# mjsargent/gym-miniworld

Measured on AMD Instinct MI355X. Metric: env-steps/s (80x60 RGB obs), higher is better.
Workload: dtype f64 sim / f32 render / u8 obs; 1 GPU; maze8192; env_id=MiniWorld-Maze-v0, envs_per_gpu=8192, global_envs=8192, obs=80x60 RGB, domain_rand=False, actions=uniform random over {turn_left, turn_right, move_forward}, counter-based, auto_reset=True, parallelism=env-sharded x1

## Files before the change

### gym_miniworld_amd/build.py

```python
import os
import subprocess
import sys

HERE = os.path.dirname(os.path.abspath(__file__))
CSRC = os.path.join(HERE, "csrc")
SOURCES = ["mwb_api.hip", "mwb_kernels.hip"]
HEADERS = ["mwb_internal.h", "mwb_glibc_trig.h", "mwb_sincos_table.inc", os.path.join("..", "..", "include", "miniworld_batch.h")]
OUT = os.path.join(HERE, "libmwbatch.so")
REMARKS = os.path.join(HERE, "libmwbatch.resources.txt")
FLAGS = ["--offload-arch=gfx950", "-O3", "-std=c++17", "-fPIC", "-shared", "-ffp-contract=off", "-Wall",
         "-Wno-unused-value"]


def needs_build():
    if not os.path.exists(OUT):
        return True
    t = os.path.getmtime(OUT)
    return any(os.path.getmtime(os.path.join(CSRC, f)) > t for f in SOURCES + HEADERS)


def source_digest():
    import hashlib
    h = hashlib.sha1()
    for f in SOURCES + HEADERS:
        with open(os.path.join(CSRC, f), "rb") as fh:
            h.update(fh.read())
    h.update(" ".join(FLAGS).encode())
    return h.hexdigest()


def build(force=False, verbose=False):
    if not force and not needs_build():
        return OUT
    hipcc = os.environ.get("HIPCC", "/opt/rocm/bin/hipcc")
    if not os.path.exists(hipcc):
        hipcc = "hipcc"
    cmd = [hipcc] + FLAGS + ["-Rpass-analysis=kernel-resource-usage", "-o", OUT] + [os.path.join(CSRC, f) for f in SOURCES]
    if verbose:
        print(" ".join(cmd))
    digest = source_digest()
    r = subprocess.run(cmd, stderr=subprocess.PIPE, text=True)
    remarks = [ln for ln in r.stderr.split("\n") if "-Rpass-analysis" in ln]
    rest = [ln for ln in r.stderr.split("\n") if "-Rpass-analysis" not in ln and ln.strip()]
    if rest:
        sys.stderr.write("\n".join(rest) + "\n")
    if r.returncode != 0:
        raise subprocess.CalledProcessError(r.returncode, cmd)
    with open(REMARKS, "w") as fh:
        fh.write("digest %s\n" % digest)
        fh.write("\n".join(remarks) + "\n")
    return OUT


if __name__ == "__main__":
    build(force="--force" in sys.argv, verbose=True)
    print("built", OUT)
```

### gym_miniworld_amd/csrc/mwb_api.hip

```cpp
#include <math.h>
#include <stdio.h>
#include <stdlib.h>
#include <string.h>

#include <string>
#include <vector>

#include "mwb_internal.h"

static thread_local std::string g_err;
static int set_err(int code, const std::string &msg) { g_err = msg; return code; }
#define HIP_TRY(expr)                                                                       \
    do {                                                                                    \
        hipError_t _e = (expr);                                                             \
        if (_e != hipSuccess)                                                               \
            return set_err(MWB_EHIP, std::string(#expr) + ": " + hipGetErrorString(_e));    \
    } while (0)

struct DevGuard {
    int prev = -1;
    hipError_t err;
    explicit DevGuard(int dev) {
        err = hipGetDevice(&prev);
        if (err == hipSuccess && prev != dev) err = hipSetDevice(dev); else if (err == hipSuccess) prev = -1;
    }
    ~DevGuard() { if (prev >= 0) (void)hipSetDevice(prev); }
};
#define USE_DEVICE(dev)                                                                             \
    DevGuard _dev_guard(dev);                                                                        \
    if (_dev_guard.err != hipSuccess)                                                                \
        return set_err(MWB_EHIP, std::string("hipSetDevice: ") + hipGetErrorString(_dev_guard.err))

struct mwb_handle {
    mwb_config cfg;
    MwbDev dev;
    std::vector<void *> allocs;
    std::vector<std::vector<uint32_t>> tex_levels[MWB_MAX_TEX];
    int tex_w[MWB_MAX_TEX], tex_h[MWB_MAX_TEX];
    uint32_t *texels_dev;
    MwbTexDesc *tex_desc_dev;
    bool seeded, textures_dirty, have_textures;
    bool have_obs;
    int *scratch_int_dev;
    bool timing, timing_now;
    int timing_period, timing_tick;
    std::vector<hipEvent_t> ev_pool;
    size_t ev_used;
    hipEvent_t *ev;
    bool overlap_reset;
    void *pack;
    size_t pack_bytes;
    void *stack;
    int stack_n, stack_dtype;
    int stack_fused;
    int stack_planes, stack_pos;
    size_t stack_bytes;
    hipStream_t side;
    hipEvent_t ev_fork, ev_join;
    struct HostMesh { bool set = false; int n_tris = 0, n_nodes = 0, n_orders = 1, tex_id = -1; float min_c[3], max_c[3]; std::vector<float> nodes, tris, tris2, shade; };
    HostMesh meshes[MWB_NUM_MESHES];
    bool meshes_dirty;
    float4 *mesh_data_dev;
    MwbMeshDesc *mesh_desc_dev;
    float *view_frame;
    bool frame_reuse;
};

extern "C" const char *mwb_last_error(void) { return g_err.c_str(); }
extern "C" int mwb_abi_version(void) { return MWB_ABI_VERSION; }

static const uint64_t K512[80] = {
    0x428a2f98d728ae22ULL, 0x7137449123ef65cdULL, 0xb5c0fbcfec4d3b2fULL, 0xe9b5dba58189dbbcULL, 0x3956c25bf348b538ULL,
    0x59f111f1b605d019ULL, 0x923f82a4af194f9bULL, 0xab1c5ed5da6d8118ULL, 0xd807aa98a3030242ULL, 0x12835b0145706fbeULL,
    0x243185be4ee4b28cULL, 0x550c7dc3d5ffb4e2ULL, 0x72be5d74f27b896fULL, 0x80deb1fe3b1696b1ULL, 0x9bdc06a725c71235ULL,
    0xc19bf174cf692694ULL, 0xe49b69c19ef14ad2ULL, 0xefbe4786384f25e3ULL, 0x0fc19dc68b8cd5b5ULL, 0x240ca1cc77ac9c65ULL,
    0x2de92c6f592b0275ULL, 0x4a7484aa6ea6e483ULL, 0x5cb0a9dcbd41fbd4ULL, 0x76f988da831153b5ULL, 0x983e5152ee66dfabULL,
    0xa831c66d2db43210ULL, 0xb00327c898fb213fULL, 0xbf597fc7beef0ee4ULL, 0xc6e00bf33da88fc2ULL, 0xd5a79147930aa725ULL,
    0x06ca6351e003826fULL, 0x142929670a0e6e70ULL, 0x27b70a8546d22ffcULL, 0x2e1b21385c26c926ULL, 0x4d2c6dfc5ac42aedULL,
    0x53380d139d95b3dfULL, 0x650a73548baf63deULL, 0x766a0abb3c77b2a8ULL, 0x81c2c92e47edaee6ULL, 0x92722c851482353bULL,
    0xa2bfe8a14cf10364ULL, 0xa81a664bbc423001ULL, 0xc24b8b70d0f89791ULL, 0xc76c51a30654be30ULL, 0xd192e819d6ef5218ULL,
    0xd69906245565a910ULL, 0xf40e35855771202aULL, 0x106aa07032bbd1b8ULL, 0x19a4c116b8d2d0c8ULL, 0x1e376c085141ab53ULL,
    0x2748774cdf8eeb99ULL, 0x34b0bcb5e19b48a8ULL, 0x391c0cb3c5c95a63ULL, 0x4ed8aa4ae3418acbULL, 0x5b9cca4f7763e373ULL,
    0x682e6ff3d6b2b8a3ULL, 0x748f82ee5defb2fcULL, 0x78a5636f43172f60ULL, 0x84c87814a1f0ab72ULL, 0x8cc702081a6439ecULL,
    0x90befffa23631e28ULL, 0xa4506cebde82bde9ULL, 0xbef9a3f7b2c67915ULL, 0xc67178f2e372532bULL, 0xca273eceea26619cULL,
    0xd186b8c721c0c207ULL, 0xeada7dd6cde0eb1eULL, 0xf57d4f7fee6ed178ULL, 0x06f067aa72176fbaULL, 0x0a637dc5a2c898a6ULL,
    0x113f9804bef90daeULL, 0x1b710b35131c471bULL, 0x28db77f523047d84ULL, 0x32caab7b40c72493ULL, 0x3c9ebe0a15c9bebcULL,
    0x431d67c49c100d4cULL, 0x4cc5d4becb3e42b6ULL, 0x597f299cfc657e2aULL, 0x5fcb6fab3ad6faecULL, 0x6c44198c4a475817ULL};

static inline uint64_t rotr64(uint64_t x, int n) { return (x >> n) | (x << (64 - n)); }

static void sha512_short(const uint8_t *msg, size_t len, uint8_t out[64]) {
// ... 229 lines not shown
    if (rc == MWB_OK && (d.exp_flags & 4)) rc = dev_alloc(h, &d.dbg_counters, (size_t)8);
    if (rc == MWB_OK) rc = dev_alloc(h, &d.cost, 2 * N);
    if (rc == MWB_OK) rc = dev_alloc(h, &d.bucket, N);
    if (rc == MWB_OK) rc = dev_alloc(h, &d.order_bufs[0], N);
    if (rc == MWB_OK) rc = dev_alloc(h, &d.order_bufs[1], N);
    if (rc == MWB_OK) rc = dev_alloc(h, &d.order_state, (size_t)2);
    if (rc == MWB_OK) {
        std::vector<int32_t> ident(N);
        for (size_t i = 0; i < N; i++) ident[i] = (int32_t)i;
        for (int k = 0; k < 2 && rc == MWB_OK; k++)
            if (hipMemcpy(d.order_bufs[k], ident.data(), N * sizeof(int32_t), hipMemcpyHostToDevice) != hipSuccess) rc = set_err(MWB_EHIP, "mwb_create: hipMemcpy failed");
    }
    if (rc != MWB_OK) { mwb_destroy(h); return rc; }
    if ((d.task == MWB_TASK_TMAZE && d.task_args[3] > 0) || (d.task == MWB_TASK_TMAZE_TWOBOX && d.task_args[0] == 0)) {
        std::vector<int64_t> ones(N, 1);
        if (hipMemcpy(d.episode_count, ones.data(), N * sizeof(int64_t), hipMemcpyHostToDevice) != hipSuccess) {
            mwb_destroy(h);
            return set_err(MWB_EHIP, "mwb_create: hipMemcpy failed");
        }
    }
    if (hipMemset(d.carrying, 0xFF, N * sizeof(int32_t)) != hipSuccess) { mwb_destroy(h); return set_err(MWB_EHIP, "mwb_create: hipMemset failed"); }
    d.tex_desc = h->tex_desc_dev;
    h->texels_dev = nullptr; d.texels = nullptr;
    h->seeded = false; h->textures_dirty = false; h->have_textures = false; h->have_obs = false;
    h->timing = false; h->timing_now = false; h->timing_period = 1; h->timing_tick = 0; h->ev_used = 0; h->ev = nullptr;
    { const char *no = getenv("MWB_NO_OVERLAP"); h->overlap_reset = !(no && atoi(no)); }
    h->side = nullptr; h->ev_fork = nullptr; h->ev_join = nullptr;
    h->view_frame = nullptr;
    h->meshes_dirty = false; h->mesh_data_dev = nullptr; d.mesh_desc = h->mesh_desc_dev; d.mesh_data = nullptr;
    h->stack = nullptr; h->stack_n = 0; h->stack_dtype = 0; h->stack_bytes = 0; h->stack_planes = 0; h->stack_pos = 0; h->stack_fused = 0;
    int prio_lo = 0, prio_hi = 0;
    hipDeviceGetStreamPriorityRange(&prio_lo, &prio_hi);
    if (hipStreamCreateWithPriority(&h->side, hipStreamNonBlocking, prio_hi) != hipSuccess ||
        hipEventCreateWithFlags(&h->ev_fork, hipEventDisableTiming) != hipSuccess ||
        hipEventCreateWithFlags(&h->ev_join, hipEventDisableTiming) != hipSuccess) {
        mwb_destroy(h);
        return set_err(MWB_EHIP, "mwb_create: could not create the side stream / events");
    }
    for (int i = 0; i < MWB_MAX_TEX; i++) { h->tex_w[i] = 0; h->tex_h[i] = 0; }
    if (d.tile_w == 0) {
        int wshift = 0;
        while ((1 << wshift) < d.W) wshift++;
        if (mwb_render_lds_bytes(d) > 160 * 1024 || ((size_t)d.H << wshift) > 65536) {
            int tw = 0, th = 0;
            mwb_view_tile(&tw, &th);
            d.tile_w = tw < d.W ? tw : d.W; d.tile_h = th < d.H ? th : d.H;
        }
    }
    { const char *no = getenv("MWB_NO_FRAME_REUSE"); h->frame_reuse = !(no && atoi(no)) && d.tile_w == 0; }
    rc = dev_alloc(h, &d.reuse_stats, (size_t)2);
    if (rc == MWB_OK && h->frame_reuse) {
        rc = dev_alloc(h, &d.frame_cache, N * d.W * d.H * 3);
        if (rc == MWB_OK && d.want_depth) rc = dev_alloc(h, &d.depth_cache, N * d.W * d.H);
        if (rc == MWB_OK) rc = dev_alloc(h, &d.frame_cached, N);
        if (rc == MWB_OK) rc = dev_alloc(h, &d.frame_same, N);
    }
    if (rc != MWB_OK) { mwb_destroy(h); return rc; }
    if (int prc = mwb_prepare_kernels(d)) {
        mwb_destroy(h);
        return set_err(prc == -2 ? MWB_EHIP : MWB_EINVAL,
                       prc == -1 ? "mwb_create: world + observation too large for the 160 KB LDS staging buffers (room table + W*H*3 frame)"
                       : prc == -3 ? "mwb_create: observation too large for the 16-bit pixel queue (H << ceil(log2 W) must not exceed 65536)"
                                   : "mwb_create: hipFuncSetAttribute(MaxDynamicSharedMemorySize) failed");
    }
    *out = h;
    return MWB_OK;
}

extern "C" int mwb_destroy(mwb_handle *h) {
    if (!h) return MWB_OK;
    DevGuard _dev_guard(h->cfg.device);
    hipDeviceSynchronize();
    for (void *p : h->allocs) hipFree(p);
    if (h->texels_dev) hipFree(h->texels_dev);
    if (h->mesh_data_dev) hipFree(h->mesh_data_dev);
    for (hipEvent_t e : h->ev_pool) hipEventDestroy(e);
    if (h->ev_fork) hipEventDestroy(h->ev_fork);
    if (h->ev_join) hipEventDestroy(h->ev_join);
    if (h->side) hipStreamDestroy(h->side);
    delete h;
    return MWB_OK;
}

static void build_mips(const uint8_t *rgb, int w, int h, std::vector<std::vector<uint32_t>> &levels) {
    levels.clear();
    std::vector<uint32_t> cur((size_t)w * h);
    for (int y = 0; y < h; y++)
        for (int x = 0; x < w; x++) {
            const uint8_t *p = rgb + ((size_t)(h - 1 - y) * w + x) * 3;
            cur[(size_t)y * w + x] = p[0] | (p[1] << 8) | (p[2] << 16) | 0xFF000000u;
        }
    levels.push_back(cur);
    int sw = w, sh = h;
    while (sw > 1 || sh > 1) {
        int dw = sw > 1 ? sw / 2 : 1, dh = sh > 1 ? sh / 2 : 1;
        std::vector<uint32_t> nxt((size_t)dw * dh);
        const std::vector<uint32_t> &src = levels.back();
        for (int j = 0; j < dh; j++) {
            int j0 = (int)(((long long)j * sh) / dh), j1 = (int)((((long long)(j + 1) * sh) + dh - 1) / dh);
            for (int i = 0; i < dw; i++) {
                int i0 = (int)(((long long)i * sw) / dw), i1 = (int)((((long long)(i + 1) * sw) + dw - 1) / dw);
                uint32_t sum[4] = {0, 0, 0, 0};
                for (int y = j0; y < j1; y++)
                    for (int x = i0; x < i1; x++) {
                        uint32_t t = src[(size_t)y * sw + x];
                        sum[0] += t & 255u; sum[1] += (t >> 8) & 255u; sum[2] += (t >> 16) & 255u; sum[3] += t >> 24;
                    }
                uint32_t cnt = (uint32_t)((j1 - j0) * (i1 - i0));
                uint32_t o = 0;
                for (int c = 0; c < 4; c++) o |= ((sum[c] + cnt / 2) / cnt) << (8 * c);
                nxt[(size_t)j * dw + i] = o;
            }
        }
        levels.push_back(nxt);
        sw = dw; sh = dh;
    }
}

extern "C" int mwb_set_texture(mwb_handle *h, int tex_id, int width, int height, const uint8_t *rgb) {
    if (!h || !rgb) return set_err(MWB_EINVAL, "mwb_set_texture: null argument");
    if (tex_id < 0 || tex_id >= MWB_MAX_TEX || width <= 0 || height <= 0 || width > 4096 || height > 4096)
        return set_err(MWB_EINVAL, "mwb_set_texture: bad texture id or size");
    build_mips(rgb, width, height, h->tex_levels[tex_id]);
    if ((int)h->tex_levels[tex_id].size() > MWB_MAX_LEVELS) return set_err(MWB_EINVAL, "mwb_set_texture: too many mip levels");
    h->tex_w[tex_id] = width; h->tex_h[tex_id] = height;
    h->textures_dirty = true;
    return MWB_OK;
}

static int upload_textures(mwb_handle *h) {
    USE_DEVICE(h->cfg.device);
    const int n_tex = h->dev.n_tex;
    for (int i = 0; i < n_tex; i++)
        if (h->tex_w[i] == 0)
            return set_err(MWB_ESTATE, "render requested before the task's " + std::to_string(n_tex) + " textures were set (mwb_set_texture)");
    std::vector<uint32_t> all;
    MwbTexDesc desc[MWB_MAX_TEX];
    memset(desc, 0, sizeof(desc));
    for (int i = 0; i < n_tex; i++) {
        desc[i].w = h->tex_w[i]; desc[i].h = h->tex_h[i]; desc[i].n_levels = (int)h->tex_levels[i].size();
        desc[i].sc_s = (float)(512.0 / h->tex_w[i]); desc[i].sc_t = (float)(512.0 / h->tex_h[i]);
        for (size_t l = 0; l < h->tex_levels[i].size(); l++) {
            desc[i].level_off[l] = (uint32_t)all.size();
            all.insert(all.end(), h->tex_levels[i][l].begin(), h->tex_levels[i][l].end());
        }
    }
    HIP_TRY(hipDeviceSynchronize());
    if (h->texels_dev) { hipFree(h->texels_dev); h->texels_dev = nullptr; }
    HIP_TRY(hipMalloc((void **)&h->texels_dev, all.size() * 4));
    HIP_TRY(hipMemcpy(h->texels_dev, all.data(), all.size() * 4, hipMemcpyHostToDevice));
    HIP_TRY(hipMemcpy(h->tex_desc_dev, desc, sizeof(desc), hipMemcpyHostToDevice));
    h->dev.texels = h->texels_dev;
    h->textures_dirty = false; h->have_textures = true;
    return MWB_OK;
}

extern "C" int mwb_set_mesh(mwb_handle *h, int geom, int n_tris, const float *verts, const float *norms, const float *texcs, int tex_slot,
                            const float *min_coords, const float *max_coords, int n_nodes, int n_orders, const float *nodes, const int32_t *perm) {
    if (!h || !verts || !norms || !texcs || !min_coords || !max_coords || !nodes || !perm) return set_err(MWB_EINVAL, "mwb_set_mesh: null argument");
    if (geom < 0 || geom >= MWB_NUM_MESHES || n_tris <= 0 || n_tris >= (1 << 24) || n_nodes <= 0 || tex_slot >= MWB_MAX_TEX || (n_orders != 1 && n_orders != 8))
        return set_err(MWB_EINVAL, "mwb_set_mesh: bad geometry id / sizes");
    for (int ord = 0; ord < n_orders; ord++) {
        std::vector<char> seen((size_t)n_tris, 0);
        const float *on = nodes + (size_t)ord * n_nodes * 8;
        for (int i = 0; i < n_nodes; i++) {
            int32_t skip, fc;
            memcpy(&skip, on + (size_t)i * 8 + 3, 4); memcpy(&fc, on + (size_t)i * 8 + 7, 4);
            const int cnt = (int)((uint32_t)fc >> 24), first = (int)((uint32_t)fc & 0xFFFFFFu);
            if (skip <= i || skip > n_nodes || first + cnt > n_tris || (cnt == 0 && i + 1 >= n_nodes))
                return set_err(MWB_EINVAL, "mwb_set_mesh: malformed hierarchy");
            for (int k = 0; k < cnt; k++) seen[(size_t)first + k] = 1;
        }
        for (int i = 0; i < n_tris; i++)
            if (!seen[i] || perm[i] < 0 || perm[i] >= n_tris) return set_err(MWB_EINVAL, "mwb_set_mesh: the leaves must cover every triangle once");
    }
    mwb_handle::HostMesh &m = h->meshes[geom];
    m.set = true; m.n_tris = n_tris; m.n_nodes = n_nodes; m.n_orders = n_orders; m.tex_id = tex_slot;
    for (int k = 0; k < 3; k++) { m.min_c[k] = min_coords[k]; m.max_c[k] = max_coords[k]; }
    m.nodes.assign(nodes, nodes + (size_t)n_orders * n_nodes * 8);
    auto rec = [&](int tri, float *o) {
        const float *v = verts + (size_t)tri * 9;
        const float e1[3] = {v[3] - v[0], v[4] - v[1], v[5] - v[2]}, e2[3] = {v[6] - v[0], v[7] - v[1], v[8] - v[2]};
        o[0] = v[0]; o[1] = v[1]; o[2] = v[2]; o[3] = e1[0]; o[4] = e1[1]; o[5] = e1[2]; o[6] = e2[0]; o[7] = e2[1]; o[8] = e2[2];
        int32_t idx = tri; memcpy(o + 9, &idx, 4); o[10] = 0; o[11] = 0;
    };
    m.tris.resize((size_t)n_tris * 12); m.tris2.resize((size_t)n_tris * 12); m.shade.assign((size_t)n_tris * 16, 0.0f);
    for (int i = 0; i < n_tris; i++) {
        rec(perm[i], &m.tris[(size_t)i * 12]);
        rec(i, &m.tris2[(size_t)i * 12]);
        float *o = &m.shade[(size_t)i * 16];
        memcpy(o, norms + (size_t)i * 9, 36);
        memcpy(o + 9, texcs + (size_t)i * 6, 24);
    }
    h->meshes_dirty = true;
    return MWB_OK;
}

extern "C" int mwb_set_mesh_dims(mwb_handle *h, int geom, double height, double scale, double radius, int is_f32) {
    if (!h) return set_err(MWB_EINVAL, "mwb_set_mesh_dims: null handle");
    if (geom < 0 || geom >= MWB_NUM_MESHES || !(height > 0) || !(scale > 0) || !(radius > 0) || !std::isfinite(scale) || !std::isfinite(radius))
        return set_err(MWB_EINVAL, "mwb_set_mesh_dims: bad argument");
    MwbDev &d = h->dev;
    int k = 0;
    while (k < d.n_mesh_dims && !(d.mesh_dims[k].geom == geom && d.mesh_dims[k].height == height)) k++;
    if (k == MWB_MAX_MESH_DIMS) return set_err(MWB_EINVAL, "mwb_set_mesh_dims: table full");
    d.mesh_dims[k].geom = geom; d.mesh_dims[k].height = height; d.mesh_dims[k].scale = scale; d.mesh_dims[k].radius = radius; d.mesh_dims[k].is_f32 = is_f32 ? 1 : 0;
    if (k == d.n_mesh_dims) d.n_mesh_dims++;
    return MWB_OK;
}

static const int *task_meshes(int task, int *n) {
    static const int pick[2] = {MWB_MESH_BALL, MWB_MESH_KEY}, health[1] = {MWB_MESH_MEDKIT}, three[3] = {MWB_MESH_DUCKIE, MWB_MESH_KEY, MWB_MESH_BALL},
                     sign[1] = {MWB_MESH_KEY}, side[2] = {MWB_MESH_BUILDING, MWB_MESH_CONE}, gap[1] = {MWB_MESH_BUILDING};
    switch (task) {
    case MWB_TASK_PICKUPOBJS: case MWB_TASK_ROOMOBJS: *n = 2; return pick;
    case MWB_TASK_COLLECTHEALTH: *n = 1; return health;
    case MWB_TASK_THREEROOMS: *n = 3; return three;
    case MWB_TASK_SIGN: *n = 1; return sign;
    case MWB_TASK_SIDEWALK: *n = 2; return side;
    case MWB_TASK_WALLGAP: *n = 1; return gap;
    }
    *n = 0; return nullptr;
}

static int upload_meshes(mwb_handle *h) {
    int n_need = 0;
    const int *need = task_meshes(h->dev.task, &n_need);
    for (int k = 0; k < n_need; k++) {
// ... 684 lines not shown
```

### gym_miniworld_amd/csrc/mwb_kernels.hip

```cpp
#include "mwb_internal.h"
#include "mwb_glibc_trig.h"

#define WAVE 64

__device__ __forceinline__ double ref_sin(double x) { return mwb_trig::in_range(x) ? mwb_trig::sin_glibc(x) : sin(x); }
__device__ __forceinline__ double ref_cos(double x) { return mwb_trig::in_range(x) ? mwb_trig::cos_glibc(x) : cos(x); }

__device__ __forceinline__ uint32_t mt_temper(uint32_t y) {
    y ^= (y >> 11);
    y ^= (y << 7) & 0x9d2c5680u;
    y ^= (y << 15) & 0xefc60000u;
    y ^= (y >> 18);
    return y;
}

__device__ __forceinline__ uint32_t mt_mix(uint32_t a, uint32_t b, uint32_t c) {
    uint32_t y = (a & 0x80000000u) | (b & 0x7fffffffu);
    return c ^ (y >> 1) ^ ((y & 1u) ? 0x9908b0dfu : 0u);
}

struct MtSerial {
    uint32_t *key;
    int pos;
    __device__ void load(uint32_t *st) { key = st; pos = (int)st[624]; }
// ... 1976 lines not shown
        float tmin = t1 < t2 ? t1 : t2, tmax = t1 < t2 ? t2 : t1;
        if (tmin > tn) { tn = tmin; face = a * 2 + (ld[a] > 0 ? 0 : 1); }
        if (tmax < tf) tf = tmax;
    }
    if (miss || face < 0 || !(tn <= tf) || !(tn > 0)) return -1;
    t_out = tn;
    return face;
}

#ifndef ENT_WGS_PER_CU
#define ENT_WGS_PER_CU 4
#endif
#define KIND_MESH 5u
#define KIND_FRAME 6u
__device__ __forceinline__ float dot3f(const float *a, const float *b) { return fmaf(a[2], b[2], fmaf(a[1], b[1], a[0] * b[0])); }
__device__ __forceinline__ void cross3f(const float *a, const float *b, float *o) {
    o[0] = fmaf(a[1], b[2], -(a[2] * b[1])); o[1] = fmaf(a[2], b[0], -(a[0] * b[2])); o[2] = fmaf(a[0], b[1], -(a[1] * b[0]));
}
__device__ __forceinline__ void mesh_local_dir(const float *blk, const float *dv, float *ld) {
    const float c = blk[FC_BOX_C], s = blk[FC_BOX_S], inv_s = blk[FC_LIT_BOX + FE_MESH_INVS];
    ld[0] = fmaf(dv[0], c, -(dv[2] * s)) * inv_s; ld[1] = dv[1] * inv_s; ld[2] = fmaf(dv[0], s, dv[2] * c) * inv_s;
}
__device__ __forceinline__ bool mesh_tri(const float *lo, const float *ld, const float4 r0, const float4 r1, const float4 r2, bool need_inside,
                                         float &t, float &u, float &v, float &det) {
    const float v0[3] = {r0.x, r0.y, r0.z}, e1[3] = {r0.w, r1.x, r1.y}, e2[3] = {r1.z, r1.w, r2.x};
    float pv[3], qv[3];
    cross3f(ld, e2, pv);
    det = dot3f(e1, pv);
    if (!(det > 0.0f)) return false;
    const float tv[3] = {lo[0] - v0[0], lo[1] - v0[1], lo[2] - v0[2]};
    u = dot3f(tv, pv);
    cross3f(tv, e1, qv);
    v = dot3f(ld, qv);
    if (need_inside && (u < 0.0f || u > det || v < 0.0f || u + v > det)) return false;
    t = dot3f(e2, qv) / det;
    return need_inside ? t > 0.0f : true;
}
#define MQ_CAP 320
#define MB_HALF 4
#define MB_TASKS 320
#define MB_WAVE_BYTES (MB_HALF * 64 * 8 + MB_TASKS * 2 + 64 * 4 + 16)
typedef float f4n __attribute__((ext_vector_type(4)));
__device__ __forceinline__ int trace_frame(const float *blk, const float *dv, float &t_out) {
    const float c = blk[FC_BOX_C], s = blk[FC_BOX_S];
    const float *fe = blk + FC_LIT_BOX;
    const float ld[3] = {fmaf(dv[0], c, -(dv[2] * s)), dv[1], fmaf(dv[0], s, dv[2] * c)};
    const float lo_[3] = {blk[FC_BOX_LO], blk[FC_BOX_LO + 1], blk[FC_BOX_LO + 2]};
    const float lo[3] = {0.0f, -fe[FE_FRAME_HY], -fe[FE_FRAME_HZ]}, hi[3] = {fe[FE_FRAME_SX], fe[FE_FRAME_HY], fe[FE_FRAME_HZ]};
    float tn = -INFINITY, tf = INFINITY;
    int face = -1;
    bool miss = false;
#pragma unroll
    for (int a = 0; a < 3; a++) {
        if (ld[a] == 0) { miss = miss || lo_[a] < lo[a] || lo_[a] > hi[a]; continue; }
        const float inv = 1.0f / ld[a];
        const float t1 = (lo[a] - lo_[a]) * inv, t2 = (hi[a] - lo_[a]) * inv;
        const float tmin = t1 < t2 ? t1 : t2, tmax = t1 < t2 ? t2 : t1;
        if (tmin > tn) { tn = tmin; face = a * 2 + (ld[a] > 0 ? 0 : 1); }
        if (tmax < tf) tf = tmax;
    }
    if (miss || face <= 0 || !(tn <= tf) || !(tn > 0)) return -1;
    t_out = tn;
    if (face != 1) return 100;
    const float z = fmaf(tn, ld[2], lo_[2]);
    const int n_ch = __float_as_int(fe[FE_FRAME_NCH]);
    int i = (int)floorf((fe[FE_FRAME_HZ] - z) / fe[FE_FRAME_CW]);
    return i < 0 ? 0 : (i >= n_ch ? n_ch - 1 : i);
}
__device__ __forceinline__ bool frame_front_tc(const float *blk, int cell, const float *dv, float &s_, float &t_) {
    const float c = blk[FC_BOX_C], s = blk[FC_BOX_S];
    const float *fe = blk + FC_LIT_BOX;
    const float ld[3] = {fmaf(dv[0], c, -(dv[2] * s)), dv[1], fmaf(dv[0], s, dv[2] * c)};
    const float lo_[3] = {blk[FC_BOX_LO], blk[FC_BOX_LO + 1], blk[FC_BOX_LO + 2]};
    const float tt = (fe[FE_FRAME_SX] - lo_[0]) / ld[0];
    const float y = fmaf(tt, ld[1], lo_[1]), z = fmaf(tt, ld[2], lo_[2]);
    const float z1 = fe[FE_FRAME_HZ] - fe[FE_FRAME_CW] * (float)cell;
    s_ = (z1 - z) / fe[FE_FRAME_CW]; t_ = (y + fe[FE_FRAME_HY]) / (2.0f * fe[FE_FRAME_HY]);
    return ld[0] != 0.0f && tt > 0.0f;
}

struct TexLds { int w, h, n_levels; float sc_s, sc_t; int pad[3]; uint32_t off[MWB_MAX_LEVELS]; };
static_assert(sizeof(TexLds) == sizeof(MwbTexDesc), "TexLds mirrors MwbTexDesc");

__device__ __forceinline__ void bilinear(const uint32_t *__restrict__ texels, uint32_t off, int w, int h, float s, float t, float *rgb) {
    float uu = fmaf(s, (float)w, -0.5f), vv = fmaf(t, (float)h, -0.5f);
    float fu = floorf(uu), fv = floorf(vv);
    float a = uu - fu, b = vv - fv;
    int i0 = (int)fu, j0 = (int)fv;
    int i1 = i0 + 1; if (i1 >= w) i1 -= w; if (i0 < 0) i0 += w;
    int j1 = j0 + 1; if (j1 >= h) j1 -= h; if (j0 < 0) j0 += h;
    const uint32_t r0 = off + __umul24((uint32_t)j0, (uint32_t)w), r1 = off + __umul24((uint32_t)j1, (uint32_t)w);
    const char *tb = (const char *)texels;
    auto texel = [tb](uint32_t idx) { return *(const uint32_t *)(tb + (size_t)(idx << 2)); };
    uint32_t t00 = texel(r0 + (uint32_t)i0), t10 = texel(r0 + (uint32_t)i1), t01 = texel(r1 + (uint32_t)i0), t11 = texel(r1 + (uint32_t)i1);
    float w00 = (1.0f - a) * (1.0f - b), w10 = a * (1.0f - b), w01 = (1.0f - a) * b, w11 = a * b;
#pragma unroll
    for (int k = 0; k < 3; k++) {
        float c00 = (float)((t00 >> (8 * k)) & 255u), c10 = (float)((t10 >> (8 * k)) & 255u);
        float c01 = (float)((t01 >> (8 * k)) & 255u), c11 = (float)((t11 >> (8 * k)) & 255u);
        rgb[k] = fmaf(c11, w11, fmaf(c01, w01, fmaf(c10, w10, c00 * w00)));
    }
}

__device__ __forceinline__ void sample_texture(const uint32_t *__restrict__ texels, const TexLds &T, float s, float t, float sx,
                                               float tx, float sy, float ty, bool valid, float *rgb) {
    const int4 dims = *(const int4 *)&T.w;
    const int maxl = dims.z - 1;
    const float fw = (float)dims.x, fh = (float)dims.y;
    const float dsdx = (sx - s) * fw, dtdx = (tx - t) * fh;
    const float dsdy = (sy - s) * fw, dtdy = (ty - t) * fh;
    const float r1 = fmaf(dsdx, dsdx, dtdx * dtdx), r2 = fmaf(dsdy, dsdy, dtdy * dtdy);
    const float rho2 = r1 > r2 ? r1 : r2;
    const float lg = 0.5f * __log2f(fmaxf(rho2, 1.0f));
    const float lambda = (valid && rho2 < INFINITY) ? lg : (float)maxl;
    float ws = s - floorf(s), wt = t - floorf(t);
    ws = (ws >= 0.0f && ws < 1.0f) ? ws : 0.0f;
    wt = (wt >= 0.0f && wt < 1.0f) ? wt : 0.0f;
    const float fl = floorf(lambda);
    int l0 = (int)fl; l0 = l0 > maxl ? maxl : l0;
    const int l1 = l0 + 1 > maxl ? maxl : l0 + 1;
    const float fr = (l0 == maxl) ? 0.0f : lambda - fl;
    float c0[3], c1[3];
    int w0 = dims.x >> l0; w0 = w0 < 1 ? 1 : w0;
    int h0 = dims.y >> l0; h0 = h0 < 1 ? 1 : h0;
    int w1 = dims.x >> l1; w1 = w1 < 1 ? 1 : w1;
    int h1 = dims.y >> l1; h1 = h1 < 1 ? 1 : h1;
    bilinear(texels, T.off[l0], w0, h0, ws, wt, c0);
    bilinear(texels, T.off[l1], w1, h1, ws, wt, c1);
#pragma unroll
    for (int k = 0; k < 3; k++) rgb[k] = fmaf(c1[k] - c0[k], fr, c0[k]);
}

__device__ __forceinline__ bool plane_texcoord(int axis, float plane, float u_org, float u_scale, float sc_t, const float *o,
                                               const float *dv, float &s, float &t) {
    float od = axis == 0 ? dv[0] : axis == 1 ? dv[1] : dv[2];
    float oo = axis == 0 ? o[0] : axis == 1 ? o[1] : o[2];
    float tt = (plane - oo) * __builtin_amdgcn_rcpf(od);
    float px = fmaf(tt, dv[0], o[0]), py = fmaf(tt, dv[1], o[1]), pz = fmaf(tt, dv[2], o[2]);
    float a = axis == 0 ? pz : px;
    float b = axis == 1 ? pz : py;
    s = (a - u_org) * u_scale; t = b * sc_t;
    return od != 0.0f && tt > 0.0f;
}

template <int NBOX, bool POLY>
struct RenderCtx {
    const float *rooms, *fc;
    const TexLds *tex;
    const uint32_t *texels;
    uint8_t *fb;
    float *depth;
    Cam cam;
    int n_rooms, cam_room, W, H, layout;
    int depth_stride;
    float cull_cc[1], cull_oc[1][3], zA, zB;
    bool boxes_in_view;
    const MwbMeshDesc *mesh_desc;
    const uint4 *mdesc;
    unsigned long long *mb_slots;
    uint16_t *mb_tasks;
    uint32_t *mb_pix;
    int *mb_count;
    const float4 *mesh_data;
    int exp_flags;
    uint32_t mesh_slots;
    unsigned long long *dbg_counters;
    const uint4 *item_res;
    int part_h_inv;
    __device__ __forceinline__ uint32_t item_boxes(int px, int py) const {
        if (NBOX == 1 || !item_res) return 0xFFFFFFFFu;
        const int item = ((px * 4370) >> 16) * 4 + ((py * part_h_inv) >> 16);
        return item_res[item].z;
    }

    __device__ __forceinline__ static void neighbour_rays_of(const Cam &cam, const float *dc, float *dx, float *dy) {
        const float sx = 2.0f * cam.invW * cam.TW, sy = 2.0f * cam.invH * cam.TH;
#pragma unroll
        for (int k = 0; k < 3; k++) { dx[k] = fmaf(cam.S[k], sx, dc[k]); dy[k] = fmaf(cam.U[k], sy, dc[k]); }
    }
    __device__ __forceinline__ void neighbour_rays(const float *dc, float *dx, float *dy) const {
        const float sx = 2.0f * cam.invW * cam.TW, sy = 2.0f * cam.invH * cam.TH;
#pragma unroll
        for (int k = 0; k < 3; k++) { dx[k] = fmaf(cam.S[k], sx, dc[k]); dy[k] = fmaf(cam.U[k], sy, dc[k]); }
    }

    template <bool PATH>
    __device__ __forceinline__ uint32_t trace_from(int room, const float *dv, float &t_hit, uint32_t &path) const {
        if constexpr (POLY) return trace_rooms_poly<PATH>(rooms, n_rooms, room, cam.eye, dv, t_hit, path);
        else return trace_rooms<PATH>(rooms, n_rooms, room, cam.eye, dv, t_hit, path);
    }
    template <bool PATH>
    __device__ __forceinline__ uint32_t trace(const float *dv, float &t_hit, uint32_t &path) const {
        return trace_from<PATH>(cam_room, dv, t_hit, path);
    }

    template <bool INTERIOR>
    __device__ __forceinline__ void shade_poly(uint32_t key, int first_k, float cx, float cy, float *col) const {
        const uint32_t kind = key & 7u, side = (key >> 3) & 3u;
        if (!INTERIOR) {
            if (kind == KIND_SKY) { col[0] = fc[FC_SKY]; col[1] = fc[FC_SKY + 1]; col[2] = fc[FC_SKY + 2]; return; }
            if (kind == KIND_BOX) {
                const float *lb = fc + FC_LIT_BOX + 3 * ((key >> 3) & 7u) + (NBOX > 1 ? (key >> 6) * FC_BOX_STRIDE : 0u);
                col[0] = lb[0]; col[1] = lb[1]; col[2] = lb[2];
                return;
            }
        }
        const float *r = rooms + __umul24(key >> 6, MWB_POLY_ROOM_WORDS);
        const float height = fabsf(r[PW_HEIGHT]);
        const uint32_t texw = (uint32_t)__float_as_int(r[PW_TEX]);
        const float *ed = r + PW_EDGE0 + __umul24(side, PW_EDGE_WORDS);
        const float4 a = *(const float4 *)ed;
// ... 1928 lines not shown
```

Baseline: 13.97 million env-steps/s.

## Store textures as precomputed 2x2 bilinear footprints for single 16-byte loads

Texture mip levels are re-laid out on the host so that each (w+1)x(h+1) entry holds the four wrapped neighbouring texels needed for bilinear filtering. The kernel then computes one index per mip level and issues one 16-byte vector load instead of four scattered 4-byte loads, and drops the wrap-around branches. This cuts memory transactions and address arithmetic in the texture sampling path. The cost is roughly four times the texture memory footprint, a new 32-bit offset limit check, and possibly lower cache hit rates.

```diff
diff --git a/gym_miniworld_amd/build.py b/gym_miniworld_amd/build.py
--- a/gym_miniworld_amd/build.py
+++ b/gym_miniworld_amd/build.py
@@ -5,7 +5,7 @@
 HERE = os.path.dirname(os.path.abspath(__file__))
 CSRC = os.path.join(HERE, "csrc")
 SOURCES = ["mwb_api.hip", "mwb_kernels.hip"]
-HEADERS = ["mwb_internal.h", "mwb_glibc_trig.h", "mwb_sincos_table.inc", os.path.join("..", "..", "include", "miniworld_batch.h")]
+HEADERS = ["mwb_internal.h", "mwb_glibc_trig.h", "mwb_sincos_table.inc", "mwb_texture_host.h", os.path.join("..", "..", "include", "miniworld_batch.h")]
 OUT = os.path.join(HERE, "libmwbatch.so")
 REMARKS = os.path.join(HERE, "libmwbatch.resources.txt")
 FLAGS = ["--offload-arch=gfx950", "-O3", "-std=c++17", "-fPIC", "-shared", "-ffp-contract=off", "-Wall",
diff --git a/gym_miniworld_amd/csrc/mwb_api.hip b/gym_miniworld_amd/csrc/mwb_api.hip
--- a/gym_miniworld_amd/csrc/mwb_api.hip
+++ b/gym_miniworld_amd/csrc/mwb_api.hip
@@ -7,6 +7,7 @@
 #include <vector>
 
 #include "mwb_internal.h"
+#include "mwb_texture_host.h"
 
 static thread_local std::string g_err;
 static int set_err(int code, const std::string &msg) { g_err = msg; return code; }
@@ -402,40 +403,6 @@
     return MWB_OK;
 }
 
-static void build_mips(const uint8_t *rgb, int w, int h, std::vector<std::vector<uint32_t>> &levels) {
-    levels.clear();
-    std::vector<uint32_t> cur((size_t)w * h);
-    for (int y = 0; y < h; y++)
-        for (int x = 0; x < w; x++) {
-            const uint8_t *p = rgb + ((size_t)(h - 1 - y) * w + x) * 3;
-            cur[(size_t)y * w + x] = p[0] | (p[1] << 8) | (p[2] << 16) | 0xFF000000u;
-        }
-    levels.push_back(cur);
-    int sw = w, sh = h;
-    while (sw > 1 || sh > 1) {
-        int dw = sw > 1 ? sw / 2 : 1, dh = sh > 1 ? sh / 2 : 1;
-        std::vector<uint32_t> nxt((size_t)dw * dh);
-        const std::vector<uint32_t> &src = levels.back();
-        for (int j = 0; j < dh; j++) {
-            int j0 = (int)(((long long)j * sh) / dh), j1 = (int)((((long long)(j + 1) * sh) + dh - 1) / dh);
-            for (int i = 0; i < dw; i++) {
-                int i0 = (int)(((long long)i * sw) / dw), i1 = (int)((((long long)(i + 1) * sw) + dw - 1) / dw);
-                uint32_t sum[4] = {0, 0, 0, 0};
-                for (int y = j0; y < j1; y++)
-                    for (int x = i0; x < i1; x++) {
-                        uint32_t t = src[(size_t)y * sw + x];
-                        sum[0] += t & 255u; sum[1] += (t >> 8) & 255u; sum[2] += (t >> 16) & 255u; sum[3] += t >> 24;
-                    }
-                uint32_t cnt = (uint32_t)((j1 - j0) * (i1 - i0));
-                uint32_t o = 0;
-                for (int c = 0; c < 4; c++) o |= ((sum[c] + cnt / 2) / cnt) << (8 * c);
-                nxt[(size_t)j * dw + i] = o;
-            }
-        }
-        levels.push_back(nxt);
-        sw = dw; sh = dh;
-    }
-}
 
 extern "C" int mwb_set_texture(mwb_handle *h, int tex_id, int width, int height, const uint8_t *rgb) {
     if (!h || !rgb) return set_err(MWB_EINVAL, "mwb_set_texture: null argument");
@@ -454,16 +421,19 @@
     for (int i = 0; i < n_tex; i++)
         if (h->tex_w[i] == 0)
             return set_err(MWB_ESTATE, "render requested before the task's " + std::to_string(n_tex) + " textures were set (mwb_set_texture)");
+    size_t total = 0;
+    for (int i = 0; i < n_tex; i++) total += pyramid_footprint_entries(h->tex_w[i], h->tex_h[i]);
+    if (total * 16 > 0xFFFFFFFFull)
+        return set_err(MWB_EINVAL, "textures too large: the footprint tables take " + std::to_string(total * 16) +
+                                       " bytes, byte offsets into them must fit 32 bits");
     std::vector<uint32_t> all;
+    all.reserve(total * 4);
     MwbTexDesc desc[MWB_MAX_TEX];
     memset(desc, 0, sizeof(desc));
     for (int i = 0; i < n_tex; i++) {
         desc[i].w = h->tex_w[i]; desc[i].h = h->tex_h[i]; desc[i].n_levels = (int)h->tex_levels[i].size();
         desc[i].sc_s = (float)(512.0 / h->tex_w[i]); desc[i].sc_t = (float)(512.0 / h->tex_h[i]);
-        for (size_t l = 0; l < h->tex_levels[i].size(); l++) {
-            desc[i].level_off[l] = (uint32_t)all.size();
-            all.insert(all.end(), h->tex_levels[i][l].begin(), h->tex_levels[i][l].end());
-        }
+        append_pyramid_footprints(h->tex_levels[i], h->tex_w[i], h->tex_h[i], desc[i].level_off, all);
     }
     HIP_TRY(hipDeviceSynchronize());
     if (h->texels_dev) { hipFree(h->texels_dev); h->texels_dev = nullptr; }
diff --git a/gym_miniworld_amd/csrc/mwb_kernels.hip b/gym_miniworld_amd/csrc/mwb_kernels.hip
--- a/gym_miniworld_amd/csrc/mwb_kernels.hip
+++ b/gym_miniworld_amd/csrc/mwb_kernels.hip
@@ -2082,17 +2082,18 @@
 struct TexLds { int w, h, n_levels; float sc_s, sc_t; int pad[3]; uint32_t off[MWB_MAX_LEVELS]; };
 static_assert(sizeof(TexLds) == sizeof(MwbTexDesc), "TexLds mirrors MwbTexDesc");
 
-__device__ __forceinline__ void bilinear(const uint32_t *__restrict__ texels, uint32_t off, int w, int h, float s, float t, float *rgb) {
+__device__ __forceinline__ uint32_t footprint_index(uint32_t off, int w, int h, float s, float t, float &a, float &b) {
     float uu = fmaf(s, (float)w, -0.5f), vv = fmaf(t, (float)h, -0.5f);
     float fu = floorf(uu), fv = floorf(vv);
-    float a = uu - fu, b = vv - fv;
+    a = uu - fu; b = vv - fv;
     int i0 = (int)fu, j0 = (int)fv;
-    int i1 = i0 + 1; if (i1 >= w) i1 -= w; if (i0 < 0) i0 += w;
-    int j1 = j0 + 1; if (j1 >= h) j1 -= h; if (j0 < 0) j0 += h;
-    const uint32_t r0 = off + __umul24((uint32_t)j0, (uint32_t)w), r1 = off + __umul24((uint32_t)j1, (uint32_t)w);
-    const char *tb = (const char *)texels;
-    auto texel = [tb](uint32_t idx) { return *(const uint32_t *)(tb + (size_t)(idx << 2)); };
-    uint32_t t00 = texel(r0 + (uint32_t)i0), t10 = texel(r0 + (uint32_t)i1), t01 = texel(r1 + (uint32_t)i0), t11 = texel(r1 + (uint32_t)i1);
+    return off + __umul24((uint32_t)(j0 + 1), (uint32_t)(w + 1)) + (uint32_t)(i0 + 1);
+}
+__device__ __forceinline__ uint4 footprint_load(const uint32_t *__restrict__ texels, uint32_t idx) {
+    return *(const uint4 *)((const char *)texels + (size_t)(idx << 4));
+}
+__device__ __forceinline__ void bilinear_blend(const uint4 fp, float a, float b, float *rgb) {
+    const uint32_t t00 = fp.x, t10 = fp.y, t01 = fp.z, t11 = fp.w;
     float w00 = (1.0f - a) * (1.0f - b), w10 = a * (1.0f - b), w01 = (1.0f - a) * b, w11 = a * b;
 #pragma unroll
     for (int k = 0; k < 3; k++) {
@@ -2125,8 +2126,12 @@
     int h0 = dims.y >> l0; h0 = h0 < 1 ? 1 : h0;
     int w1 = dims.x >> l1; w1 = w1 < 1 ? 1 : w1;
     int h1 = dims.y >> l1; h1 = h1 < 1 ? 1 : h1;
-    bilinear(texels, T.off[l0], w0, h0, ws, wt, c0);
-    bilinear(texels, T.off[l1], w1, h1, ws, wt, c1);
+    float a0, b0, a1, b1;
+    const uint32_t e0 = footprint_index(T.off[l0], w0, h0, ws, wt, a0, b0);
+    const uint32_t e1 = footprint_index(T.off[l1], w1, h1, ws, wt, a1, b1);
+    const uint4 f0 = footprint_load(texels, e0), f1 = footprint_load(texels, e1);
+    bilinear_blend(f0, a0, b0, c0);
+    bilinear_blend(f1, a1, b1, c1);
 #pragma unroll
     for (int k = 0; k < 3; k++) rgb[k] = fmaf(c1[k] - c0[k], fr, c0[k]);
 }
diff --git a/gym_miniworld_amd/csrc/mwb_texture_host.h b/gym_miniworld_amd/csrc/mwb_texture_host.h
--- /dev/null
+++ b/gym_miniworld_amd/csrc/mwb_texture_host.h
@@ -0,0 +1,73 @@
+#pragma once
+#include <stddef.h>
+#include <stdint.h>
+
+#include <vector>
+
+static inline void build_mips(const uint8_t *rgb, int w, int h, std::vector<std::vector<uint32_t>> &levels) {
+    levels.clear();
+    std::vector<uint32_t> cur((size_t)w * h);
+    for (int y = 0; y < h; y++)
+        for (int x = 0; x < w; x++) {
+            const uint8_t *p = rgb + ((size_t)(h - 1 - y) * w + x) * 3;
+            cur[(size_t)y * w + x] = p[0] | (p[1] << 8) | (p[2] << 16) | 0xFF000000u;
+        }
+    levels.push_back(cur);
+    int sw = w, sh = h;
+    while (sw > 1 || sh > 1) {
+        int dw = sw > 1 ? sw / 2 : 1, dh = sh > 1 ? sh / 2 : 1;
+        std::vector<uint32_t> nxt((size_t)dw * dh);
+        const std::vector<uint32_t> &src = levels.back();
+        for (int j = 0; j < dh; j++) {
+            int j0 = (int)(((long long)j * sh) / dh), j1 = (int)((((long long)(j + 1) * sh) + dh - 1) / dh);
+            for (int i = 0; i < dw; i++) {
+                int i0 = (int)(((long long)i * sw) / dw), i1 = (int)((((long long)(i + 1) * sw) + dw - 1) / dw);
+                uint32_t sum[4] = {0, 0, 0, 0};
+                for (int y = j0; y < j1; y++)
+                    for (int x = i0; x < i1; x++) {
+                        uint32_t t = src[(size_t)y * sw + x];
+                        sum[0] += t & 255u; sum[1] += (t >> 8) & 255u; sum[2] += (t >> 16) & 255u; sum[3] += t >> 24;
+                    }
+                uint32_t cnt = (uint32_t)((j1 - j0) * (i1 - i0));
+                uint32_t o = 0;
+                for (int c = 0; c < 4; c++) o |= ((sum[c] + cnt / 2) / cnt) << (8 * c);
+                nxt[(size_t)j * dw + i] = o;
+            }
+        }
+        levels.push_back(nxt);
+        sw = dw; sh = dh;
+    }
+}
+
+static inline size_t footprint_entries(int w, int h) { return (size_t)(w + 1) * (size_t)(h + 1); }
+
+static inline void append_footprints(const uint32_t *L, int w, int h, std::vector<uint32_t> &out) {
+    size_t o = out.size();
+    out.resize(o + 4 * footprint_entries(w, h));
+    for (int J = 0; J <= h; J++) {
+        const int j0 = (J - 1 + h) % h, j1 = J % h;
+        const uint32_t *r0 = L + (size_t)j0 * w, *r1 = L + (size_t)j1 * w;
+        for (int I = 0; I <= w; I++) {
+            const int i0 = (I - 1 + w) % w, i1 = I % w;
+            out[o++] = r0[i0]; out[o++] = r0[i1]; out[o++] = r1[i0]; out[o++] = r1[i1];
+        }
+    }
+}
+
+static inline size_t pyramid_footprint_entries(int w, int h) {
+    size_t n = 0;
+    for (;;) {
+        n += footprint_entries(w, h);
+        if (w == 1 && h == 1) return n;
+        w = w > 1 ? w / 2 : 1; h = h > 1 ? h / 2 : 1;
+    }
+}
+
+static inline void append_pyramid_footprints(const std::vector<std::vector<uint32_t>> &levels, int w, int h, uint32_t *level_off,
+                                             std::vector<uint32_t> &all) {
+    for (size_t l = 0; l < levels.size(); l++) {
+        level_off[l] = (uint32_t)(all.size() / 4);
+        append_footprints(levels[l].data(), w, h, all);
+        w = w > 1 ? w / 2 : 1; h = h > 1 ? h / 2 : 1;
+    }
+}
```

After: 14.49 million env-steps/s, median of 6. +3.7%, better.
